# muonzoo/cutesdr

Measured on AMD Instinct MI355X. Metric: complex IQ MSamples/s through CFastFIR+demod chain; achieved HBM GB/s vs peak, higher is better.
Workload: dtype f32; 1 GPU; C3: 256 channels/GPU x 2^19 IQ samples, 16384-pt CFastFIR overlap-save (8193 taps, hop 8192), shared -5..+5 kHz filter @62.5 kS/s; channels_per_gpu=256, samples_per_channel=524288, fft_size=16384, parallelism=channels sharded x1, no data-path collective

## Files before the change

### __graft_entry__.py

```python
import os
import sys

ROOT = os.path.dirname(os.path.abspath(__file__))
if ROOT not in sys.path:
    sys.path.insert(0, ROOT)


def build():
    from cutesdr_amd import _build, _capi
    lib = _build.build()
    assert os.path.exists(lib)
    assert os.path.exists(_build.alt_lib(*_build.TWREG3))
    assert os.path.exists(_build.alt_lib(*_build.PWRES0))
    from oracle import oracle as orc
    orc.build()
    from oracle import ref
    ref.build()
    import ctypes
    L = ctypes.CDLL(lib)
    missing = [n for n in _capi.declared_symbols() if not hasattr(L, n)]
    assert not missing, missing
    import cutesdr_amd


def smoke():
    import numpy as np
    import cutesdr_amd as ca
    from oracle import oracle as orc
    n, C, fs = 16384, 4, 62500.0
    T = 3 * (n // 2)
    rng = np.random.default_rng(0)
    x = 3000.0 * (rng.standard_normal((C, T)) + 1j * rng.standard_normal((C, T)))
    b = ca.FastFirBatch(C, n, device=0)
    b.setup(-5000, 5000, 0, fs)
    y = b.process(x)
    for c in range(C):
        ff = orc.CFastFIR(n)
        ff.SetupParameters(-5000, 5000, 0, fs)
        ref = ff.ProcessData(x[c])
        err = np.abs(y[c] - ref).max()
        assert err <= 2e-5 * np.abs(x[c]).max(), err
    print("smoke ok: fastfir 16384-pt x %d channels, max err %.3g" % (C, err))


if __name__ == "__main__":
    build()
    if "--smoke" in sys.argv:
        smoke()
```

### cutesdr_amd/_build.py

```python
import glob
import os
import shutil
import subprocess
import sys

HERE = os.path.dirname(os.path.abspath(__file__))
CSRC = os.path.join(HERE, "csrc")
OBJ = os.path.join(HERE, "_obj")
LIB = os.path.join(HERE, "libcutesdr_mi.so")
ARCH = "gfx950"
FLAGS = ["-O3", "-std=c++17", "-fPIC", "--offload-arch=" + ARCH, "-Wall", "-Wno-unused-function"] + \
    os.environ.get("CSDR_EXTRA_HIPCC_FLAGS", "").split()
FILE_FLAGS = {"fastfir2_kernels.hip": ["-mllvm", "-amdgpu-sched-strategy=max-ilp"] + os.environ.get("CSDR_K1_FLAGS", "").split(), "fastfir_kernels.hip": ["-mllvm", "-amdgpu-sched-strategy=max-ilp"],
              "spectrum_kernels.hip": ["-mllvm", "-amdgpu-sched-strategy=max-ilp"]}


def _difference(text):
    import re
    m = re.fullmatch(r"\(?\s*([0-9.]+)\s*-\s*([0-9.]+)\s*\)?", text.strip())
    if not m:
        raise ValueError("unexpected threshold expression in csdr_hb_taps.h: %r" % text)
    return float(m.group(1)) - float(m.group(2))


# ... 139 lines not shown
                    r[4].kill()
                raise RuntimeError("hipcc failed on %s:\n%s" % (src, out.decode(errors="replace")))
            with open(stamp, "w") as f:
                f.write(flags)

    for src, obj, extra, stamp, flags in todo:
        reap(JOBS - 1)
        cmd = [hipcc] + FLAGS + FILE_FLAGS.get(os.path.basename(src), []) + extra + ["-c", src, "-o", obj]
        if verbose:
            print(" ".join(cmd), file=sys.stderr)
        p = subprocess.Popen(cmd, stdout=subprocess.PIPE, stderr=subprocess.STDOUT)
        running.append((src, obj, stamp, flags, p))
        procs.append(obj)
    reap(0)
    if force or procs or _newer(LIB, objs):
        cmd = [hipcc, "-shared", "-fPIC", "--offload-arch=" + ARCH, "-o", LIB] + list(link_extra) + objs
        subprocess.check_call(cmd)
    return LIB


def alt_path(name):
    return os.path.join(HERE, "libcutesdr_mi_%s.so" % name)


def alt_lib(name, extra, units=("fastfir2_kernels",), verbose=False):
    build(verbose=verbose)
    hipcc = _hipcc()
    headers = glob.glob(os.path.join(CSRC, "*.h")) + glob.glob(os.path.join(CSRC, "*.hpp")) + \
        glob.glob(os.path.join(HERE, "..", "include", "*.h"))
    out = alt_path(name)
    alt, fresh = [], False
    for unit in units:
        src = os.path.join(CSRC, unit + ".hip")
        obj = os.path.join(OBJ, "%s.%s.o" % (unit, name))
        cmd = [hipcc] + FLAGS + FILE_FLAGS.get(unit + ".hip", []) + ["-I", OBJ] + list(extra) + ["-c", src, "-o", obj]
        stamp, flags = obj + ".flags", " ".join(cmd[1:-4])
        if _newer(obj, [src] + headers) or not os.path.exists(stamp) or open(stamp).read() != flags:
            if verbose:
                print(" ".join(cmd), file=sys.stderr)
            subprocess.check_call(cmd)
            with open(stamp, "w") as f:
                f.write(flags)
            fresh = True
        alt.append(obj)
    objs = [o for o in sorted(glob.glob(os.path.join(OBJ, "*.hip.o")) + glob.glob(os.path.join(OBJ, "downconv_plan_*.o")))
            if os.path.basename(o)[:-6] not in units]
    if fresh or _newer(out, objs + alt):
        subprocess.check_call([hipcc, "-shared", "-fPIC", "--offload-arch=" + ARCH, "-o", out] + objs + alt)
    return out


TWREG3 = ("twreg3", ["-DK1_TWREG=3"])
PWRES0 = ("pwres0", ["-DK1_PWRES=0"])


if __name__ == "__main__":
    kind = next((a.split("=", 1)[1] for a in sys.argv if a.startswith("--sanitize=")), None)
    var = next((a.split("=", 1)[1] for a in sys.argv if a.startswith("--variant=")), None)
    print(build(force="--force" in sys.argv, verbose=True, sanitize=kind, variant=var,
                variant_flags=[a for a in sys.argv[1:] if a.startswith("-D")]))
```

### cutesdr_amd/csrc/capi_fastfir.hip

```cpp
#include "capi_common.hpp"
#include "capi_internal.hpp"
#include <algorithm>
#include "fastfir_kernels.h"
#include "fastfir_design_kernels.h"
#include "host_math.hpp"
#include "patch_queue.hpp"
#include <cmath>
#include <cstdlib>
#include <cstring>
#include <vector>

using namespace csdr;

static int log2_of(int n)
{
    int l = 0;
    while ((1 << l) < n) l++;
    return ((1 << l) == n) ? l : -1;
}

struct csdr_fastfir_batch {
    int device, channels, n, log2n;
    int cus;
    hipStream_t last_stream;
// ... 377 lines not shown
    else {
        b->last_kernel = FASTFIR_KERNEL_NONE;
        CSDR_HIP(fastfir_launch(b->log2n, a, s));
        b->last_kernel = FASTFIR_KERNEL_GENERIC;
    }
    b->hist_cur ^= 1;
    return CSDR_OK;
}

int csdr__fastfir_batch_copy_row(csdr_fastfir_batch *dst, int dr, csdr_fastfir_batch *src, int sr)
{
    if (!dst || !src || dst->n != src->n || dr < 0 || dr >= dst->channels || sr < 0 || sr >= src->channels)
        return fail(CSDR_EINVAL, "bad argument");
    if (!device_ok(dst->device)) return CSDR_EHIP;
    CSDR_HIP(hipDeviceSynchronize());
    const int L = dst->n / 2;
    const size_t shalf = (size_t)src->channels * L * 2, dhalf = (size_t)dst->channels * L * 2;
    CSDR_HIP(hipMemcpy(dst->d_hist + dst->hist_cur * dhalf + (size_t)dr * L * 2,
                       src->d_hist + src->hist_cur * shalf + (size_t)sr * L * 2, (size_t)L * 8, hipMemcpyDeviceToDevice));
    const int sslot = src->per_channel ? sr : 0;
    { const int rcm = fetch_mirror(src, sslot); if (rcm) return rcm; }
    const std::vector<cd> &H = src->resp[sslot];
    if (dst->channels > 1 && !dst->per_channel) return fail(CSDR_ESTATE, "destination rows share one filter");
    const int slot = dst->per_channel ? dr : 0;
    int rc = set_response(dst, slot, H);
    if (rc) return rc;
    dst->own_design = dst->own_design && src->own_design;
    dst->flo = dst->fhi = dst->off = dst->fs = std::nan("");
    return CSDR_OK;
}

int csdr__fastfir_set_variant(csdr_fastfir_batch *b, int variant)
{
    if (!b || (variant != 0 && variant != 2)) return CSDR_EINVAL;
    b->variant = variant;
    return CSDR_OK;
}

int csdr__fastfir_set_own_design(csdr_fastfir_batch *b, int own)
{
    if (!b) return CSDR_EINVAL;
    b->own_design = own != 0;
    return CSDR_OK;
}

int csdr__fastfir_last_kernel(const csdr_fastfir_batch *b, int *kernel, int *twreg)
{
    if (!b || !kernel || !twreg) return CSDR_EINVAL;
    *kernel = b->last_kernel;
    *twreg = fastfir2_twreg();
    return CSDR_OK;
}

int csdr__dbg_fastfir_stage(csdr_fastfir_batch *b, int stage, float *d_dbg)
{
    if (!b) return CSDR_EINVAL;
    b->dbg_stage = stage; b->dbg_out = d_dbg;
    return CSDR_OK;
}

}

struct csdr_fastfir {
    csdr_fastfir_batch *b;
    int n, pending;
    PinnedBuf pin_in, pin_out;
    hipStream_t s = nullptr;
    float *d_in, *d_out;
    size_t cap;
};

static int ensure_cap(csdr_fastfir *f, size_t samples)
{
    if (samples <= f->cap) return CSDR_OK;
    if (f->d_in) (void)hipFree(f->d_in);
    if (f->d_out) (void)hipFree(f->d_out);
    f->d_in = f->d_out = nullptr; f->cap = 0;
    CSDR_HIP(hipMalloc((void **)&f->d_in, samples * 8));
    CSDR_HIP(hipMalloc((void **)&f->d_out, samples * 8));
    f->cap = samples;
    return CSDR_OK;
}

extern "C" {

csdr_fastfir *csdr_fastfir_create(int device, int fft_size)
{
    csdr_fastfir_batch *b = csdr_fastfir_batch_create(device, 1, fft_size);
    if (!b) return nullptr;
    csdr_fastfir *f = new csdr_fastfir();
    f->b = b; f->n = fft_size; f->pending = 0; f->d_in = f->d_out = nullptr; f->cap = 0;
    if (hipStreamCreateWithFlags(&f->s, hipStreamNonBlocking) != hipSuccess) { csdr_fastfir_destroy(f); fail(CSDR_EHIP, "stream creation failed"); return nullptr; }
    return f;
}

void csdr_fastfir_destroy(csdr_fastfir *f)
{
    if (!f) return;
    (void)hipSetDevice(f->b->device);
    if (f->d_in) (void)hipFree(f->d_in);
    if (f->d_out) (void)hipFree(f->d_out);
    if (f->s) { (void)hipStreamSynchronize(f->s); (void)hipStreamDestroy(f->s); }
    csdr_fastfir_batch_destroy(f->b);
    delete f;
}

// ... 37 lines not shown
```

### cutesdr_amd/csrc/capi_hosttest.hip

```cpp
#include "capi_common.hpp"
#include "host_math.hpp"
#include "dc_host.hpp"
#include "pc_host.hpp"
#include "display_plan.hpp"
#include "testgen_host.hpp"
#include "scope_host.hpp"
#include "plotter_host.hpp"
#include "seq_host.hpp"
#include "spurcal_host.hpp"
#include "nb_host.hpp"
#include "fastfir_kernels.h"
#include "fft_core.hpp"
#include <cstring>

using namespace csdr;

template <int SIGN> static void host_head4_gain(const float *x4, const float *g4, float *out4)
{
    v2f x[4];
    for (int q = 0; q < 4; q++) x[q] = v2f{x4[2 * q], x4[2 * q + 1]};
    dit_head4_gain<0, 4, SIGN>(x, v2f{g4[0], g4[1]}, v2f{g4[2], g4[3]});
    for (int q = 0; q < 4; q++) { out4[2 * q] = x[q].x; out4[2 * q + 1] = x[q].y; }
}
template <int R, int SIGN> static void host_dft_middle(const float *in, float *out)
// ... 10 lines not shown
    int done = -1;
    static_for<0, R / 4>([&](auto I) {
        if (I.value != i) return;
        constexpr int Q = R / 4;
        v2f x[R];
        for (int p = 0; p < R; p++) x[p] = v2f{0.0f, 0.0f};
        for (int q = 0; q < 4; q++) x[I.value + q * Q] = v2f{in4[2 * q], in4[2 * q + 1]};
        if (middle) dit_tail_middle_r4<I.value, R, SIGN>(x); else dit_tail_r4<I.value, R, SIGN>(x);
        for (int q = 0; q < 4; q++) { out4[2 * q] = x[I.value + q * Q].x; out4[2 * q + 1] = x[I.value + q * Q].y; }
        done = 0;
    });
    return done;
}
template <int R, int SIGN> static void host_dft_r4(int middle, const float *in, float *out)
{
    v2f x[R];
    for (int n = 0; n < R; n++) x[bitrev<R>(n)] = v2f{in[2 * n], in[2 * n + 1]};
    static_for<0, R / 4>([&](auto G) { dit_head4<G.value, R, SIGN>(x); });
    if constexpr (R == 32) dit_single<8, 32, SIGN>(x);
    if (middle) {
        static_for<0, R / 4>([&](auto I) { dit_tail_middle_r4<I.value, R, SIGN>(x); });
        for (int r = 0; r < R / 2; r++) { out[2 * r] = x[R / 4 + r].x; out[2 * r + 1] = x[R / 4 + r].y; }
    } else {
        static_for<0, R / 4>([&](auto I) { dit_tail_r4<I.value, R, SIGN>(x); });
        for (int r = 0; r < R; r++) { out[2 * r] = x[r].x; out[2 * r + 1] = x[r].y; }
    }
}

extern "C" {

int csdr__host_dit_tail_r4(int r, int sign, int i, int middle, const float *in4, float *out4)
{
    if (r == 16) return sign > 0 ? host_tail_r4<16, +1>(i, middle, in4, out4) : host_tail_r4<16, -1>(i, middle, in4, out4);
    if (r == 32) return sign > 0 ? host_tail_r4<32, +1>(i, middle, in4, out4) : host_tail_r4<32, -1>(i, middle, in4, out4);
    return -1;
}
int csdr__host_dft_r4(int r, int sign, int middle, const float *in, float *out)
{
    if (r == 16 && sign > 0) host_dft_r4<16, +1>(middle, in, out);
    else if (r == 16) host_dft_r4<16, -1>(middle, in, out);
    else if (r == 32 && sign > 0) host_dft_r4<32, +1>(middle, in, out);
    else if (r == 32) host_dft_r4<32, -1>(middle, in, out);
    else return -1;
    return 0;
}
int csdr__host_tw_factors(int k, int sign, double *m, double *tau)
{
    const TwFactors f = tw_factors(k, sign);
    *m = f.m; *tau = f.tau;
    return f.rot;
}
int csdr__host_fastfir2_radix4(void) { return fastfir2_radix4(); }
int csdr__host_fastfir2_pwres(void) { return fastfir2_pwres(); }

int csdr__host_fastfir_design(int n, double flo, double fhi, double off, double fs, double *h_out)
{
    std::vector<cd> H;
    if (!fastfir_design(n, flo, fhi, off, fs, H)) return -1;
    memcpy(h_out, H.data(), sizeof(cd) * n);
    return 0;
}
int csdr__host_design_job(double flo, double fhi, double off, double fs, double *nfc, double *nfs)
{
    return fastfir_design_job(flo, fhi, off, fs, *nfc, *nfs) ? 0 : -1;
}
int csdr__host_fastfir_bin_of(int log2n, int t, int r) { return fastfir_bin_of(log2n, t, r); }
int csdr__host_fastfir_gains(int n, double flo, double fhi, double off, double fs, double *h_out, double *p_out)
{
    std::vector<cd> H;
    if (!fastfir_design(n, flo, fhi, off, fs, H)) return -1;
    memcpy(h_out, H.data(), sizeof(cd) * n);
    for (int k = 0; k < n; k++) p_out[k] = fastfir_gain(H[k], k);
    return 0;
}
int csdr__host_fastfir2_bin_of(int log2n, int t, int j, int e) { return fastfir2_bin_of(log2n, t, j, e); }
int csdr__host_fastfir2_gain_bin_of(int log2n, int t, int i, int c) { return fastfir2_gain_bin_of(log2n, t, i, c); }
int csdr__host_fastfir2_slot_bin(int log2n, int t, int j, int e) { return fastfir2_slot_bin(log2n, t, j, e); }
int csdr__host_fastfir2_gain_slot_bin(int log2n, int t, int i, int c) { return fastfir2_gain_slot_bin(log2n, t, i, c); }
void csdr__host_fastfir2_twshare_shift(int log2n, int t, int *inner, int *outer) { fastfir2_twshare_shift(log2n, t, inner, outer); }
int csdr__host_fastfir2_twshare(void) { return fastfir2_twshare(); }

void csdr__host_dit_head4_gain(int sign, const float *x4, const float *g4, float *out4)
{
    if (sign > 0) host_head4_gain<+1>(x4, g4, out4); else host_head4_gain<-1>(x4, g4, out4);
}
int csdr__host_dft_middle(int r, int sign, const float *in, float *out)
{
    if (r == 16 && sign > 0) host_dft_middle<16, +1>(in, out);
    else if (r == 16) host_dft_middle<16, -1>(in, out);
    else if (r == 32 && sign > 0) host_dft_middle<32, +1>(in, out);
    else if (r == 32) host_dft_middle<32, -1>(in, out);
    else return -1;
    return 0;
}

int csdr__host_dc_plan(double in_rate, double bw, int *codes, double *out_rate, int *warmup)
{
    DcPlan p = dc_make_plan(in_rate, bw);
    for (int i = 0; i < p.nstages; i++) codes[i] = p.kind[i];
    *out_rate = p.out_rate; *warmup = p.W;
    return p.nstages;
}
int csdr__host_dc_stage_taps(double in_rate, double bw, int s, double *h)
{
    DcPlan p = dc_make_plan(in_rate, bw);
    if (s < 0 || s >= p.nstages) return -1;
// ... 320 lines not shown
```

### cutesdr_amd/csrc/fastfir2_kernels.hip

```cpp
#define CSDR_FMA_BFLY 1
#define CSDR_PLAIN_CONST_FMA 1
#include "launch_once.hpp"
#include "fastfir_dev.hpp"
#include "fastfir_kernels.h"

namespace csdr {

#ifndef K1_LDAUX
#define K1_LDAUX 2
#endif
#ifndef K1_STAUX
#define K1_STAUX 2
#endif
#ifndef K1_HREG
#define K1_HREG 8
#endif
#ifndef K1_TWREG
#define K1_TWREG 16
#endif
#ifndef K1_HREG4K
#define K1_HREG4K 4
#endif
#ifndef K1_W1_FETCH_MAX_R0
#define K1_W1_FETCH_MAX_R0 2
#endif
#ifndef K1_HREG2K
#define K1_HREG2K 8
#endif
#ifndef K1_RADIX4
#define K1_RADIX4 1
#endif
#ifndef K1_PWRES
#define K1_PWRES 1
#endif
static_assert(K1_TWREG >= 0 && K1_TWREG <= 16, "K1_TWREG");

#define CSDR_SB() __builtin_amdgcn_sched_barrier(0)

#define CSDR_PRIO(p) __builtin_amdgcn_s_setprio(p)

#ifdef CSDR_K1_STAMPS
#define CSDR_STAMP(i)                                                                         \
    do {                                                                                      \
        CSDR_SB();                                                                            \
        unsigned long long now_;                                                              \
        asm volatile("s_memtime %0\n\ts_waitcnt lgkmcnt(0)" : "=s"(now_)::"memory");         \
        CSDR_SB();                                                                            \
        acc_[i] += now_ - last_;                                                              \
        last_ = now_;                                                                         \
    } while (0)
#define CSDR_STAMP_PARAMS , unsigned long long (&acc_)[16], unsigned long long &last_
#define CSDR_STAMP_ARGS , acc_, last_
#else
#define CSDR_STAMP(i) do { } while (0)
#define CSDR_STAMP_PARAMS
#define CSDR_STAMP_ARGS
#endif

template <int I> using int_c = std::integral_constant<int, I>;

template <int NG, class Compute, class Store> __device__ __forceinline__ void one_group_behind(Compute &&compute, Store &&store)
{
    static_for<0, NG + 1>([&](auto I) {
        constexpr int i = I.value;
        if constexpr (i < NG) compute(I);
        if constexpr (i > 0) {
            CSDR_STORE_GROUP_BEGIN();
            store(int_c<i - 1>{});
            CSDR_STORE_GROUP_END();
        } else {
            CSDR_SB();
        }
    });
}
template <int NG, class Compute, class Store> __device__ __forceinline__ void one_group_behind_st8(Compute &&compute, Store &&store)
{
    static_for<0, NG + 1>([&](auto I) {
        constexpr int i = I.value;
        if constexpr (i < NG) compute(I);
        if constexpr (i > 0) store(int_c<i - 1>{});
        CSDR_SB();
    });
}

constexpr int tws_group(int step) { return step < 2 ? 4 * step : ((step & 1) ? 8 - step / 2 : step / 2); }
constexpr int tws_set(int step) { return step < 2 ? step : 1 + step / 2; }
constexpr bool tws_opens(int step) { return step < 2 || (step & 1) == 0; }
constexpr int tws_row(int set, int slot)
{
    if (set < 2) return slot < 2 ? 8 - 4 * set + 8 * slot : 0;
    const int m = set - 1;
    return slot == 0 ? m : (slot == 1 ? m + 8 : (slot == 2 ? 8 - m : 16 - m));
}
constexpr int tws_row_of(int k1) { return k1 <= 16 ? k1 : 32 - k1; }
constexpr int tws_set_of(int k1)
{
    const int r = tws_row_of(k1) & 7;
    return r == 0 ? 0 : (r == 4 ? 1 : 1 + (r < 4 ? r : 8 - r));
}
constexpr int tws_slot_of(int k1)
{
    for (int slot = 0; slot < 4; slot++)
        if (tws_row(tws_set_of(k1), slot) == tws_row_of(k1)) return slot;
    return -1;
}
static_assert(tws_group(2) == 1 && tws_group(3) == 7 && tws_group(7) == 5 && tws_set(7) == 4 && tws_set_of(31) == 2 &&
              tws_slot_of(24) == 0 && tws_slot_of(16) == 1 && tws_slot_of(20) == 1 && tws_slot_of(25) == 2 && tws_slot_of(23) == 1,
              "twiddle sets of the 16384-point kernels");

template <int LOG2N, bool RG = false>
struct K1Cfg {
    using Base = FastFirCfg<LOG2N>;
    static_assert(!RG || LOG2N == 14, "the quarter-block shift is whole rows of the outer pass at N = 16384 only");
    static constexpr int VW = LOG2N == 12 ? 2 : (LOG2N == 11 ? 4 : 1);
    static constexpr int TV = Base::T;
    static constexpr int T = VW * TV;
    static constexpr int LDS_BYTES = (VW * Base::LDS_DATA + 1024) * 8;

    static constexpr int N = Base::N, R0 = Base::R0, G = Base::G, L = N / 2, HALF = R0 / 2;
    static_assert(R0 == 16 || R0 == 8 || R0 == 4 || R0 == 2, "the grouped outer pass is written for N = 2048 ... 16384");
    static constexpr int PSTEP = 2 * TV, PSTEP_LDS = PSTEP + 2 * (PSTEP / 32), PSTEP_B = PSTEP * 8;
    static constexpr int OUTER_ROW = 1024 + 2 * (1024 / 32);
    static constexpr bool TWS = LOG2N == 14;
    static constexpr int PWN = R0 == 16 ? R0 / 2 + 1 : R0;
    static constexpr bool W1_RESIDENT = R0 > K1_W1_FETCH_MAX_R0;
    static constexpr int HREG = RG ? 0 : (LOG2N == 12 ? K1_HREG4K : (LOG2N == 11 ? K1_HREG2K : K1_HREG));
    static constexpr int TWREG = RG ? K1_TWREG : 0;
    static constexpr bool R4 = RG && K1_RADIX4 != 0;
    static constexpr bool PW_RESIDENT = RG && K1_PWRES != 0;

    using Y = v2f[G][R0];
    using W1 = v2f[R0 > 2 ? G : 1];
    using Pw = v2f[G][PWN];
    using Hv = v4f[RG ? 1 : 16];
    using Pv = v4f[RG ? 8 : 1];
    using Twr = v2f[TWREG > 0 ? TWREG : 1];
};

struct K1Half { v2f v[16]; };

struct K1Thread {
    int t, voff;
    v2f *col;
    const v2f *twc;
    v2f *rowp;
    v2f *outer;
    const v2f_h *tw1;
    int nblocks;
    rsrc_t r_in, r_h, r_out;
#ifdef K1_ABLATE
    v4f habl;
    v2f twabl;
#endif
};

#ifdef K1_ABLATE
__device__ __forceinline__ void keep_alive(v4f v) { asm volatile("" ::"v"(v)); }
#endif

template <int LOG2N> __device__ __forceinline__ void k1_block_barrier()
{
#ifdef ABL_BAR
    wave_sync();
#else
    if constexpr (LOG2N == 11) wave_sync();
    else __syncthreads();
#endif
}

template <int LOG2N, bool RG, int K1> __device__ __forceinline__ v2f k1_pass_tw(const K1Thread &c, const typename K1Cfg<LOG2N, RG>::Twr &twr)
{
#ifdef ABL_TW
    return c.twabl;
#else
    if constexpr (K1 <= K1Cfg<LOG2N, RG>::TWREG) return twr[K1 - 1];
    else return lds_ld8(c.twc + 32 * K1);
#endif
}

template <int LOG2N, int J> __device__ __forceinline__ void k1_fetch_h(const K1Thread &c, typename K1Cfg<LOG2N>::Hv &hv)
{
#ifdef ABL_H
    hv[J] = c.habl;
#else
    if constexpr (J >= K1Cfg<LOG2N>::HREG) hv[J] = buf_load16(c.r_h, c.t * 16, J * (K1Cfg<LOG2N>::TV * 16));
#endif
}

template <int LOG2N> __device__ __forceinline__ void k1_store_out(const K1Thread &c, int voff, int soff, v4f v)
{
#ifdef ABL_GST
    if constexpr (LOG2N == 14) { keep_alive(v); return; }
#endif
    buf_store16_aux<K1_STAUX>(c.r_out, voff, soff, v);
}

template <int LOG2N> __device__ __forceinline__ void k1_load_half(rsrc_t r, int voff, int soff, v2f (&dst)[16])
{
    using Cfg = K1Cfg<LOG2N>;
#pragma unroll
    for (int n1 = 0; n1 < Cfg::HALF; n1++)
#pragma unroll
        for (int pp = 0; pp < Cfg::G / 2; pp++) {
            v4f v = buf_load16_aux<K1_LDAUX>(r, voff + pp * Cfg::PSTEP_B, soff + n1 * 8192);
            dst[(2 * pp) * Cfg::HALF + n1] = v2f{v.x, v.y};
            dst[(2 * pp + 1) * Cfg::HALF + n1] = v2f{v.z, v.w};
        }
}

template <int LOG2N> __device__ __forceinline__ v4f k1_w_pair(const K1Thread &c, int pp)
{
    return *reinterpret_cast<const v4f *>(c.tw1 + K1Cfg<LOG2N>::PSTEP * pp + 2 * c.t);
}
template <int LOG2N> __device__ __forceinline__ void k1_load_w1(const K1Thread &c, typename K1Cfg<LOG2N>::W1 &w1)
{
    if constexpr (K1Cfg<LOG2N>::R0 > 2) {
#pragma unroll
        for (int pp = 0; pp < K1Cfg<LOG2N>::G / 2; pp++) { const v4f v = k1_w_pair<LOG2N>(c, pp); w1[2 * pp] = v2f{v.x, v.y}; w1[2 * pp + 1] = v2f{v.z, v.w}; }
    }
}

template <int LOG2N, bool RG> __device__ __forceinline__ void k1_f1_rows16(const K1Thread &c, typename K1Cfg<LOG2N>::Y &y, typename K1Cfg<LOG2N>::Pw &pw)
{
    using Cfg = K1Cfg<LOG2N>;
    constexpr int R0 = Cfg::R0;
    v4f wv[16];
    one_group_behind<R0 / 4>([&](auto Ii) {
        constexpr int i = Ii.value;
        dit_tail_sel<K1Cfg<LOG2N, RG>::R4, i, R0, +1>(y[0]);
        dit_tail_sel<K1Cfg<LOG2N, RG>::R4, i, R0, +1>(y[1]);
        static_for<0, 4>([&](auto P) {
            constexpr int k0 = i + 4 * P.value;
            if constexpr (k0 > R0 / 2) {
                y[0][k0] = cmul_conj(y[0][k0], pw[0][R0 - k0]);
                y[1][k0] = cmul_conj(y[1][k0], pw[1][R0 - k0]);
            } else if constexpr (k0 != 0) {
                y[0][k0] = cmul(y[0][k0], pw[0][k0]);
                y[1][k0] = cmul(y[1][k0], pw[1][k0]);
            }
            wv[k0] = store_operand(y[0][k0], y[1][k0]);
        });
    }, [&](auto Ii) {
        static_for<0, 4>([&](auto P) {
            constexpr int k0 = Ii.value + 4 * P.value;
            *reinterpret_cast<v4f *>(c.outer + Cfg::OUTER_ROW * k0) = wv[k0];
        });
    });
}
template <int LOG2N> __device__ __forceinline__ void k1_f1_rows2(const K1Thread &c, typename K1Cfg<LOG2N>::Y &y)
{
    using Cfg = K1Cfg<LOG2N>;
    v4f wv[16], wq[8];
    static_for<0, 8>([&](auto PP) { wq[PP.value] = k1_w_pair<LOG2N>(c, PP.value); });
    one_group_behind<4>([&](auto Ii) {
        static_for<0, 2>([&](auto Q) {
            constexpr int pp = 2 * Ii.value + Q.value;
            y[2 * pp][1] = cmul(y[2 * pp][1], v2f{wq[pp].x, wq[pp].y});
            y[2 * pp + 1][1] = cmul(y[2 * pp + 1][1], v2f{wq[pp].z, wq[pp].w});
            wv[pp] = store_operand(y[2 * pp][0], y[2 * pp + 1][0]);
            wv[8 + pp] = store_operand(y[2 * pp][1], y[2 * pp + 1][1]);
// ... 2 lines not shown
        static_for<0, 2>([&](auto Q) {
            constexpr int pp = 2 * Ii.value + Q.value;
            *reinterpret_cast<v4f *>(c.outer + Cfg::PSTEP_LDS * pp) = wv[pp];
            *reinterpret_cast<v4f *>(c.outer + Cfg::OUTER_ROW + Cfg::PSTEP_LDS * pp) = wv[8 + pp];
        });
    });
}
template <int LOG2N> __device__ __forceinline__ void k1_f1_rows84(const K1Thread &c, typename K1Cfg<LOG2N>::Y &y, typename K1Cfg<LOG2N>::Pw &pw)
{
    using Cfg = K1Cfg<LOG2N>;
    constexpr int R0 = Cfg::R0, G = Cfg::G, NG = 4, RPG = R0 / NG;
    v4f wv[16];
    one_group_behind<NG>([&](auto Ii) {
        constexpr int i = Ii.value;
        if constexpr (R0 == 8)
            static_for<0, G>([&](auto E) { bfly_dit<4 * i, +1>(y[E.value][i], y[E.value][i + 4]); });
        static_for<0, RPG>([&](auto P) {
            constexpr int k0 = i + NG * P.value;
            static_for<0, G>([&](auto E) {
                if constexpr (k0 != 0) y[E.value][k0] = cmul(y[E.value][k0], pw[E.value][k0]);
            });
            static_for<0, G / 2>([&](auto PP) {
                wv[k0 * (G / 2) + PP.value] = store_operand(y[2 * PP.value][k0], y[2 * PP.value + 1][k0]);
            });
        });
    }, [&](auto Ii) {
        static_for<0, RPG>([&](auto P) {
            constexpr int k0 = Ii.value + NG * P.value;
            static_for<0, G / 2>([&](auto PP) {
                *reinterpret_cast<v4f *>(c.outer + Cfg::OUTER_ROW * k0 + Cfg::PSTEP_LDS * PP.value) = wv[k0 * (G / 2) + PP.value];
            });
        });
    });
}
template <int LOG2N, bool RG> __device__ __forceinline__ void k1_pass_f1(const K1Thread &c, int b, K1Half &oldh, K1Half &newh, typename K1Cfg<LOG2N>::Pw &pw)
{
    using Cfg = K1Cfg<LOG2N>;
    constexpr int R0 = Cfg::R0, G = Cfg::G, HALF = Cfg::HALF;
    typename Cfg::Y y;
    static_for<0, HALF>([&](auto N1) {
        static_for<0, G>([&](auto E) {
            constexpr int e = E.value, n1 = N1.value, po = bitrev<R0>(n1), pn = bitrev<R0>(HALF + n1);
            y[e][po] = oldh.v[e * HALF + n1]; y[e][pn] = newh.v[e * HALF + n1];
        });
    });
    if constexpr (R0 == 2) {
        static_for<0, G>([&](auto E) { bfly_dit<0, +1>(y[E.value][0], y[E.value][1]); });
    } else {
        static_for<0, (R0 >= 8 ? R0 / 4 : 1)>([&](auto Gg) {
            static_for<0, G>([&](auto E) { dit_head4<Gg.value, R0, +1>(y[E.value]); });
        });
    }
    CSDR_SB();
    k1_load_half<LOG2N>(c.r_in, c.voff, (b + 1 < c.nblocks ? b + 1 : c.nblocks - 1) * (Cfg::L * 8), oldh.v);
    CSDR_SB();
    CSDR_PRIO(0);
    if constexpr (R0 == 16) k1_f1_rows16<LOG2N, RG>(c, y, pw);
    else if constexpr (R0 == 2) k1_f1_rows2<LOG2N>(c, y);
    else k1_f1_rows84<LOG2N>(c, y, pw);
}

template <int LOG2N, bool RG>
__device__ __forceinline__ void k1_f2_tail_shared(const K1Thread &c, v2f (&x)[32], typename K1Cfg<LOG2N, RG>::Hv &hv,
                                                  const typename K1Cfg<LOG2N, RG>::Twr &twr CSDR_STAMP_PARAMS)
{
    v2f tw[5][4];
    auto load_set = [&](auto S) {
        static_for<0, 4>([&](auto Q) {
            constexpr int row = tws_row(S.value, Q.value);
            if constexpr (row != 0) tw[S.value][Q.value] = k1_pass_tw<LOG2N, RG, row>(c, twr);
        });
    };
    load_set(int_c<0>{});
    CSDR_SB();
    CSDR_STAMP(8);
    one_group_behind_st8<8>([&](auto St) {
        constexpr int s = St.value, i = tws_group(s);
        if constexpr (s < 7 && tws_opens(s + 1)) load_set(int_c<tws_set(s + 1)>{});
        if constexpr (!RG) { k1_fetch_h<LOG2N, 2 * s>(c, hv); k1_fetch_h<LOG2N, 2 * s + 1>(c, hv); }
        dit_tail_sel<K1Cfg<LOG2N, RG>::R4, i, 32, +1>(x);
        static_for<0, 4>([&](auto P) {
            constexpr int k1 = i + 8 * P.value;
            if constexpr (k1 != 0 && k1 <= 16) x[k1] = cmul(x[k1], tw[tws_set_of(k1)][tws_slot_of(k1)]);
            if constexpr (k1 > 16) x[k1] = cmul_conj(x[k1], tw[tws_set_of(k1)][tws_slot_of(k1)]);
        });
    }, [&](auto St) {
        static_for<0, 4>([&](auto P) {
            constexpr int k1 = tws_group(St.value) + 8 * P.value;
            lds_st8(c.col + 34 * k1, x[k1]);
        });
    });
}
template <int LOG2N, bool RG>
__device__ __forceinline__ void k1_f2_tail_plain(const K1Thread &c, v2f (&x)[32], typename K1Cfg<LOG2N, RG>::Hv &hv,
                                                 const typename K1Cfg<LOG2N, RG>::Twr &twr CSDR_STAMP_PARAMS)
{
    v2f tw[2][4];
    static_for<1, 4>([&](auto P) { tw[0][P.value] = k1_pass_tw<LOG2N, RG, 8 * P.value>(c, twr); });
    CSDR_SB();
    CSDR_STAMP(8);
    one_group_behind_st8<8>([&](auto Ii) {
        constexpr int i = Ii.value;
        if constexpr (i < 7)
            static_for<0, 4>([&](auto P) { tw[(i + 1) & 1][P.value] = k1_pass_tw<LOG2N, RG, i + 1 + 8 * P.value>(c, twr); });
        if constexpr (!RG) { k1_fetch_h<LOG2N, 2 * i>(c, hv); k1_fetch_h<LOG2N, 2 * i + 1>(c, hv); }
        dit_tail<i, 32, +1>(x);
        static_for<0, 4>([&](auto P) {
// ... 235 lines not shown
            constexpr int g = Gg.value;
            static_for<0, G>([&](auto E) {
                constexpr int e = E.value;
                if constexpr (R0 == 16) {
                    constexpr int ka = bitrev<R0>(4 * g), kb = bitrev<R0>(4 * g + 1), kc = bitrev<R0>(4 * g + 2), kd = bitrev<R0>(4 * g + 3);
                    constexpr int H0 = R0 / 2;
                    dit_head4_seltw<g, R0, -1, g == 0, (ka <= H0), (kb <= H0), (kc <= H0), (kd <= H0)>(
                        y[e], pw[e][ka <= H0 ? ka : R0 - ka], pw[e][kb <= H0 ? kb : R0 - kb],
                        pw[e][kc <= H0 ? kc : R0 - kc], pw[e][kd <= H0 ? kd : R0 - kd]);
                } else
                    dit_head4_conjtw<g, R0, -1, g == 0>(y[e], pw[e][bitrev<R0>(4 * g)], pw[e][bitrev<R0>(4 * g + 1)],
                                                        pw[e][bitrev<R0>(4 * g + 2)], pw[e][bitrev<R0>(4 * g + 3)]);
            });
            if constexpr ((g & 1) == 1) CSDR_SB();
        });
    }
    CSDR_PRIO(2);
    if constexpr (R0 == 16) k1_i3_rows16<LOG2N, RG>(c, b, y);
    else if constexpr (R0 == 2) k1_i3_rows2<LOG2N>(c, b, y);
    else k1_i3_rows84<LOG2N>(c, b, y);
}

template <int LOG2N, bool RG> __device__ __forceinline__ void fastfir_os2_body(const FastFirArgs a)
{
    CSDR_WG_TRACE_SCOPE(a.trace, WGT_FF);
    using Cfg = K1Cfg<LOG2N, RG>;
    constexpr int N = Cfg::N, T = Cfg::TV, G = Cfg::G, L = Cfg::L, HALF = Cfg::HALF, VW = Cfg::VW;
    extern __shared__ __attribute__((aligned(16))) unsigned char smem_raw[];
    const int t = VW == 1 ? (int)threadIdx.x : (int)threadIdx.x % T, vw = VW == 1 ? 0 : (int)threadIdx.x / T;
    v2f *lds = reinterpret_cast<v2f *>(smem_raw) + vw * Cfg::Base::LDS_DATA;
    v2f *tw2 = reinterpret_cast<v2f *>(smem_raw) + VW * Cfg::Base::LDS_DATA;
    if constexpr (VW > 1) {
        for (int i = threadIdx.x; i < 1024; i += VW * T) tw2[i] = a.tw2[i];
        __syncthreads();
    }

    int wg = blockIdx.x * VW + vw, ch, run;
    if ((a.channels & 7) == 0) {
        int xcd = wg & 7, slot = wg >> 3;
        ch = (slot / a.runs) * 8 + xcd;
        run = slot % a.runs;
    } else {
        ch = wg / a.runs;
        run = wg % a.runs;
    }
    const int b0 = run * a.blocks_per_run;
    int b1 = b0 + a.blocks_per_run;
    if (b1 > a.nblocks) b1 = a.nblocks;
#if defined(__HIP_DEVICE_COMPILE__) && !defined(__gfx950__)
#error "fastfir_os2_kernel<12> relies on gfx950's s_barrier ignoring terminated waves (two virtual workgroups per workgroup)"
#endif
    if (ch >= a.channels || b0 >= b1) return;

    if constexpr (VW == 1)
        for (int i = t; i < 1024; i += T) tw2[i] = a.tw2[i];

    K1Thread c;
    c.t = t; c.tw1 = a.tw1; c.nblocks = a.nblocks;
    c.r_in = make_rsrc(a.in + (long)ch * a.in_stride, (unsigned)a.nblocks * L * 8u);
    const rsrc_t r_hist = make_rsrc(a.hist + (long)ch * L, L * 8u);
    c.r_out = make_rsrc(a.out + (long)ch * a.out_stride, (unsigned)a.nblocks * L * 8u);
    c.r_h = make_rsrc(a.h + (long)ch * a.h_stride, N * 8u);
    const rsrc_t r_g = make_rsrc(a.gain + (long)ch * (a.h_stride / 2), N * 4u);
    c.voff = t * 16;

    typename Cfg::W1 w1;
    k1_load_w1<LOG2N>(c, w1);
    typename Cfg::Pw pw;
    if constexpr (Cfg::R0 > 2) {
#pragma unroll
        for (int e = 0; e < G; e++) twiddle_powers<Cfg::PWN>(opaque(w1[e]), pw[e]);
    }

    typename Cfg::Hv hv;
#pragma unroll
    for (int j = 0; j < Cfg::HREG; j++) hv[j] = buf_load16(c.r_h, t * 16, j * (T * 16));
    typename Cfg::Pv pv;
    if constexpr (RG) {
#pragma unroll
        for (int i = 0; i < 8; i++) pv[i] = buf_load16(r_g, t * 16, i * (T * 16));
    }
#ifdef K1_ABLATE
    c.habl = v4f{1.0f, 0.0f, 1.0f, 0.0f};
    asm volatile("" : "+v"(c.habl));
    c.twabl = v2f{0.8f, 0.6f};
    asm volatile("" : "+v"(c.twabl));
#endif
    v2f x[32];
    K1Half hp, hq;
    if (b0 == 0) k1_load_half<LOG2N>(r_hist, c.voff, 0, hp.v);
    else k1_load_half<LOG2N>(c.r_in, c.voff, (b0 - 1) * (L * 8), hp.v);
    k1_load_half<LOG2N>(c.r_in, c.voff, b0 * (L * 8), hq.v);

    const int sb = t >> 5, sn = t & 31;
    c.col = lds + lds_pad(1024 * sb) + sn;
    c.twc = tw2 + sn;
    typename Cfg::Twr twr;
#pragma unroll
    for (int k1 = 1; k1 <= Cfg::TWREG; k1++) twr[k1 - 1] = a.tw2[32 * k1 + sn];
    c.rowp = lds + 34 * t;
    c.outer = lds + lds_pad(2 * t);

#ifdef K1_CYC
    const unsigned long long cyc0_ = __builtin_amdgcn_s_memtime(), rt0_ = __builtin_amdgcn_s_memrealtime();
#endif
#ifdef CSDR_K1_STAMPS
    unsigned long long acc_[16] = {0, 0, 0, 0, 0, 0, 0, 0, 0, 0, 0, 0, 0, 0, 0, 0}, last_;
    asm volatile("s_memtime %0\n\ts_waitcnt lgkmcnt(0)" : "=s"(last_)::"memory");
#endif
    auto one_block = [&](const int b, K1Half &oldh, K1Half &newh) {
        CSDR_SB();
        CSDR_PRIO(1);
        k1_pass_f1<LOG2N, RG>(c, b, oldh, newh, pw);
        CSDR_STAMP(0);
        k1_block_barrier<LOG2N>();
        CSDR_STAMP(1);
        CSDR_PRIO(3);
        k1_pass_f2<LOG2N, RG>(c, x, hv, twr CSDR_STAMP_ARGS);
        CSDR_STAMP(2);
        wave_sync();
        CSDR_PRIO(2);
        k1_pass_f3<LOG2N, RG>(c, x, hv, pv);
        CSDR_STAMP(3);
        wave_sync();
        CSDR_PRIO(0);
        k1_pass_i2<LOG2N, RG>(c, x, twr);
        CSDR_STAMP(4);
        k1_block_barrier<LOG2N>();
        CSDR_STAMP(5);
        CSDR_PRIO(3);
        k1_pass_i3<LOG2N, RG>(c, b, w1, pw);
        CSDR_STAMP(6);
    };
    __builtin_amdgcn_s_waitcnt(0x0f70);
    int b = b0;
    for (; b + 1 < b1; b += 2) {
        one_block(b, hp, hq);
        one_block(b + 1, hq, hp);
    }
    const bool odd_tail = b < b1;
    if (odd_tail) one_block(b, hp, hq);

#ifdef K1_CYC
    if (a.dbg && t == 0) {
        unsigned long long *o = reinterpret_cast<unsigned long long *>(a.dbg) + (long)blockIdx.x * 2;
        o[0] = __builtin_amdgcn_s_memtime() - cyc0_;
        o[1] = __builtin_amdgcn_s_memrealtime() - rt0_;
    }
#endif
#ifdef CSDR_K1_STAMPS
    if (a.dbg && (c.t & 63) == 0) {
        unsigned long long *o = reinterpret_cast<unsigned long long *>(a.dbg) + ((long)blockIdx.x * (T / 64) + (c.t >> 6)) * 16;
        for (int i = 0; i < 16; i++) o[i] = acc_[i];
    }
#endif
    if (b1 == a.nblocks) {
        const rsrc_t r_hn = make_rsrc(a.hist_next + (long)ch * L, L * 8u);
        v4f sv[8];
#pragma unroll
        for (int n1 = 0; n1 < HALF; n1++)
#pragma unroll
            for (int pp = 0; pp < G / 2; pp++)
                sv[n1 * (G / 2) + pp] = odd_tail ? store_operand(hq.v[(2 * pp) * HALF + n1], hq.v[(2 * pp + 1) * HALF + n1])
                                                 : store_operand(hp.v[(2 * pp) * HALF + n1], hp.v[(2 * pp + 1) * HALF + n1]);
        CSDR_STORE_GROUP_BEGIN();
#pragma unroll
        for (int n1 = 0; n1 < HALF; n1++)
#pragma unroll
            for (int pp = 0; pp < G / 2; pp++) buf_store16(r_hn, c.voff + pp * Cfg::PSTEP_B, n1 * 8192, sv[n1 * (G / 2) + pp]);
        CSDR_STORE_GROUP_END();
    }
}


template <int LOG2N>
__global__ __launch_bounds__(K1Cfg<LOG2N>::T) __attribute__((amdgpu_waves_per_eu(2, 2)))
void fastfir_os2_kernel(FastFirArgs a)
{
    fastfir_os2_body<LOG2N, LOG2N == 14>(a);
}
__global__ __launch_bounds__(K1Cfg<14>::T) __attribute__((amdgpu_waves_per_eu(2, 2)))
void fastfir_os2h_kernel(FastFirArgs a)
{
    fastfir_os2_body<14, false>(a);
}

template <int LOG2N>
static hipError_t launch2_one(const FastFirArgs &a, hipStream_t stream, int *which)
{
    using Cfg = K1Cfg<LOG2N>;
    void (*kernel)(FastFirArgs) = &fastfir_os2_kernel<LOG2N>;
    if (LOG2N == 14 && !a.gain) kernel = &fastfir_os2h_kernel;
    if (which) *which = (LOG2N == 14 && kernel != &fastfir_os2h_kernel) ? FASTFIR_KERNEL_PIPELINED_GAIN : FASTFIR_KERNEL_PIPELINED_H;
    hipError_t e = kernel == &fastfir_os2h_kernel ? CSDR_MAX_LDS_ONCE(&fastfir_os2h_kernel, Cfg::LDS_BYTES)
                                                  : CSDR_MAX_LDS_ONCE(&fastfir_os2_kernel<LOG2N>, Cfg::LDS_BYTES);
    if (e != hipSuccess) return e;
#ifdef CSDR_WG_TRACE
    FastFirArgs b = a;
    b.trace = wgtrace_next();
    hipLaunchKernelGGL(kernel, dim3((a.channels * a.runs + Cfg::VW - 1) / Cfg::VW), dim3(Cfg::T), Cfg::LDS_BYTES, stream, b);
    return hipGetLastError();
#endif
    hipLaunchKernelGGL(kernel, dim3((a.channels * a.runs + Cfg::VW - 1) / Cfg::VW), dim3(Cfg::T), Cfg::LDS_BYTES, stream, a);
    return hipGetLastError();
}

hipError_t fastfir2_launch(int log2n, const FastFirArgs &a, hipStream_t stream, int *kernel)
{
    switch (log2n) {
    case 11: return launch2_one<11>(a, stream, kernel);
    case 12: return launch2_one<12>(a, stream, kernel);
    case 13: return launch2_one<13>(a, stream, kernel);
    case 14: return launch2_one<14>(a, stream, kernel);
    default: return hipErrorInvalidValue;
    }
}

int fastfir2_twreg() { return K1_TWREG; }
int fastfir2_radix4() { return K1Cfg<14, true>::R4 ? 1 : 0; }
int fastfir2_pwres() { return K1Cfg<14, true>::PW_RESIDENT ? 1 : 0; }

int fastfir2_bin_of(int log2n, int t, int j, int e)
{
    const int R0 = (1 << log2n) / 1024;
    const int i = j >> 1, h = j & 1;
    const int k2 = i + 8 * h + 16 * e;
    return (t >> 5) + R0 * ((t & 31) + 32 * k2);
}
int fastfir2_gain_bin_of(int log2n, int t, int i, int c)
{
    return fastfir2_bin_of(log2n, t, 2 * i + (c >> 1), c & 1);
}

int fastfir2_twshare() { return 2; }
void fastfir2_twshare_shift(int log2n, int t, int *inner, int *outer)
{
    *inner = (log2n == 14 && (t & 31) >= 17) ? 1 : 0;
    *outer = (log2n == 14 && (t >> 5) > 8) ? 1 : 0;
}
int fastfir2_slot_bin(int log2n, int t, int j, int e)
{
    const int R0 = (1 << log2n) / 1024;
    int inner, outer;
    fastfir2_twshare_shift(log2n, t, &inner, &outer);
    const int k2 = ((j >> 1) + 8 * (j & 1) + 16 * e - inner) & 31;
    const int sub = ((t & 31) + 32 * k2 - outer) & 1023;
    return (t >> 5) + R0 * sub;
}
int fastfir2_gain_slot_bin(int log2n, int t, int i, int c)
{
    return fastfir2_slot_bin(log2n, t, 2 * i + (c >> 1), c & 1);
}

}
```

### cutesdr_amd/csrc/fastfir_kernels.h

```cpp
#pragma once
#include <hip/hip_runtime.h>
#include "wg_trace.hpp"

namespace csdr {

typedef float v2f_h __attribute__((ext_vector_type(2)));
typedef float v4f_h __attribute__((ext_vector_type(4)));

struct FastFirArgs {
    const v2f_h *in;
    const v2f_h *hist;
    v2f_h *hist_next;
    v2f_h *out;
    const v4f_h *h;
    const v4f_h *gain;
    const v2f_h *tw1;
    const v2f_h *tw2;
    long in_stride;
    long out_stride;
    long h_stride;
    int channels;
    int nblocks;
    int blocks_per_run;
    int runs;
    int dbg_stage;
    v2f_h *dbg;
#ifdef CSDR_WG_TRACE
    WgTraceArg trace;
#endif
};

hipError_t fastfir_launch(int log2n, const FastFirArgs &a, hipStream_t stream);
int fastfir_bin_of(int log2n, int t, int r);

enum FastFirKernel { FASTFIR_KERNEL_NONE = -1, FASTFIR_KERNEL_GENERIC = 0, FASTFIR_KERNEL_PIPELINED_H = 1, FASTFIR_KERNEL_PIPELINED_GAIN = 2 };
hipError_t fastfir2_launch(int log2n, const FastFirArgs &a, hipStream_t stream, int *kernel = nullptr);
int fastfir2_twreg();
int fastfir2_radix4();
int fastfir2_pwres();
int fastfir2_bin_of(int log2n, int t, int j, int e);
int fastfir2_gain_bin_of(int log2n, int t, int i, int c);
int fastfir2_twshare();
void fastfir2_twshare_shift(int log2n, int t, int *inner, int *outer);
int fastfir2_slot_bin(int log2n, int t, int j, int e);
int fastfir2_gain_slot_bin(int log2n, int t, int i, int c);

}
```

Baseline: 233,900 MSamples/s.

## Spread next-block prefetch across FFT passes and clamp loads at run end

Splits the next-block input prefetch into four quarters, each issued between FFT passes, so HBM loads overlap compute more evenly. With RUNEND on, the kernel stores the history tail inside the block loop and sizes the input resource so loads past the run end return zero, instead of re-reading a clamped block. It also adds optional flags that move twiddle loading into a prologue and drop the tw2 LDS table. The extra SB barriers and register pressure could hurt scheduling.

```diff
diff --git a/__graft_entry__.py b/__graft_entry__.py
--- a/__graft_entry__.py
+++ b/__graft_entry__.py
@@ -12,6 +12,8 @@
     assert os.path.exists(lib)
     assert os.path.exists(_build.alt_lib(*_build.TWREG3))
     assert os.path.exists(_build.alt_lib(*_build.PWRES0))
+    assert os.path.exists(_build.alt_lib(*_build.RUNEND0))
+    assert os.path.exists(_build.alt_lib(*_build.HBMALL))
     from oracle import oracle as orc
     orc.build()
     from oracle import ref
diff --git a/cutesdr_amd/_build.py b/cutesdr_amd/_build.py
--- a/cutesdr_amd/_build.py
+++ b/cutesdr_amd/_build.py
@@ -215,6 +215,9 @@
 
 TWREG3 = ("twreg3", ["-DK1_TWREG=3"])
 PWRES0 = ("pwres0", ["-DK1_PWRES=0"])
+HBM_KNOBS = ("K1_RUNEND", "K1_PROLOGUE", "K1_TW2LDS", "K1_LDSPREAD")
+RUNEND0 = ("runend0", ["-D%s=0" % k for k in HBM_KNOBS])
+HBMALL = ("hbmall", ["-D%s=1" % k for k in HBM_KNOBS])
 
 
 if __name__ == "__main__":
diff --git a/cutesdr_amd/csrc/capi_fastfir.hip b/cutesdr_amd/csrc/capi_fastfir.hip
--- a/cutesdr_amd/csrc/capi_fastfir.hip
+++ b/cutesdr_amd/csrc/capi_fastfir.hip
@@ -453,6 +453,16 @@
     return CSDR_OK;
 }
 
+int csdr__fastfir_read_history(csdr_fastfir_batch *b, float *out, int *cur)
+{
+    if (!b || !out || !cur) return CSDR_EINVAL;
+    if (!device_ok(b->device)) return CSDR_EHIP;
+    CSDR_HIP(hipDeviceSynchronize());
+    CSDR_HIP(hipMemcpy(out, b->d_hist, 2 * (size_t)b->channels * (b->n / 2) * 8, hipMemcpyDeviceToHost));
+    *cur = b->hist_cur;
+    return CSDR_OK;
+}
+
 int csdr__dbg_fastfir_stage(csdr_fastfir_batch *b, int stage, float *d_dbg)
 {
     if (!b) return CSDR_EINVAL;
diff --git a/cutesdr_amd/csrc/capi_hosttest.hip b/cutesdr_amd/csrc/capi_hosttest.hip
--- a/cutesdr_amd/csrc/capi_hosttest.hip
+++ b/cutesdr_amd/csrc/capi_hosttest.hip
@@ -86,6 +86,8 @@
 }
 int csdr__host_fastfir2_radix4(void) { return fastfir2_radix4(); }
 int csdr__host_fastfir2_pwres(void) { return fastfir2_pwres(); }
+int csdr__host_fastfir2_hbm_knobs(void) { return fastfir2_hbm_knobs(); }
+int csdr__host_fastfir2_gain_lds_bytes(void) { return fastfir2_gain_lds_bytes(); }
 
 int csdr__host_fastfir_design(int n, double flo, double fhi, double off, double fs, double *h_out)
 {
diff --git a/cutesdr_amd/csrc/fastfir2_kernels.hip b/cutesdr_amd/csrc/fastfir2_kernels.hip
--- a/cutesdr_amd/csrc/fastfir2_kernels.hip
+++ b/cutesdr_amd/csrc/fastfir2_kernels.hip
@@ -32,6 +32,18 @@
 #endif
 #ifndef K1_PWRES
 #define K1_PWRES 1
+#endif
+#ifndef K1_RUNEND
+#define K1_RUNEND 1
+#endif
+#ifndef K1_PROLOGUE
+#define K1_PROLOGUE 0
+#endif
+#ifndef K1_TW2LDS
+#define K1_TW2LDS 0
+#endif
+#ifndef K1_LDSPREAD
+#define K1_LDSPREAD 1
 #endif
 static_assert(K1_TWREG >= 0 && K1_TWREG <= 16, "K1_TWREG");
 
@@ -115,7 +127,6 @@
     static constexpr int VW = LOG2N == 12 ? 2 : (LOG2N == 11 ? 4 : 1);
     static constexpr int TV = Base::T;
     static constexpr int T = VW * TV;
-    static constexpr int LDS_BYTES = (VW * Base::LDS_DATA + 1024) * 8;
 
     static constexpr int N = Base::N, R0 = Base::R0, G = Base::G, L = N / 2, HALF = R0 / 2;
     static_assert(R0 == 16 || R0 == 8 || R0 == 4 || R0 == 2, "the grouped outer pass is written for N = 2048 ... 16384");
@@ -128,6 +139,11 @@
     static constexpr int TWREG = RG ? K1_TWREG : 0;
     static constexpr bool R4 = RG && K1_RADIX4 != 0;
     static constexpr bool PW_RESIDENT = RG && K1_PWRES != 0;
+    static constexpr bool TW2_LDS = !(RG && TWREG == 16 && K1_TW2LDS != 0);
+    static constexpr int LDS_BYTES = (VW * Base::LDS_DATA + (TW2_LDS ? 1024 : 0)) * 8;
+    static constexpr bool RUNEND = LOG2N == 14 && K1_RUNEND != 0;
+    static constexpr bool PROLOGUE = LOG2N == 14 && K1_PROLOGUE != 0;
+    static constexpr bool LDSPREAD = RG && K1_LDSPREAD != 0;
 
     using Y = v2f[G][R0];
     using W1 = v2f[R0 > 2 ? G : 1];
@@ -148,6 +164,10 @@
     const v2f_h *tw1;
     int nblocks;
     rsrc_t r_in, r_h, r_out;
+    const void *in;
+    unsigned in_bytes;
+    int run_end;
+    rsrc_t r_hn;
 #ifdef K1_ABLATE
     v4f habl;
     v2f twabl;
@@ -195,17 +215,46 @@
     buf_store16_aux<K1_STAUX>(c.r_out, voff, soff, v);
 }
 
-template <int LOG2N> __device__ __forceinline__ void k1_load_half(rsrc_t r, int voff, int soff, v2f (&dst)[16])
-{
-    using Cfg = K1Cfg<LOG2N>;
-#pragma unroll
-    for (int n1 = 0; n1 < Cfg::HALF; n1++)
+template <int LOG2N, int N1A = 0, int N1B = K1Cfg<LOG2N>::HALF>
+__device__ __forceinline__ void k1_load_half(rsrc_t r, int voff, int soff, v2f (&dst)[16])
+{
+    using Cfg = K1Cfg<LOG2N>;
+#pragma unroll
+    for (int n1 = N1A; n1 < N1B; n1++)
 #pragma unroll
         for (int pp = 0; pp < Cfg::G / 2; pp++) {
             v4f v = buf_load16_aux<K1_LDAUX>(r, voff + pp * Cfg::PSTEP_B, soff + n1 * 8192);
             dst[(2 * pp) * Cfg::HALF + n1] = v2f{v.x, v.y};
             dst[(2 * pp + 1) * Cfg::HALF + n1] = v2f{v.z, v.w};
         }
+}
+struct K1Next { rsrc_t r; int soff; };
+template <int LOG2N> __device__ __forceinline__ K1Next k1_next_half(const K1Thread &c, int b)
+{
+    using Cfg = K1Cfg<LOG2N>;
+    if constexpr (Cfg::RUNEND) {
+        const bool more = b + 1 < c.run_end;
+        return K1Next{make_rsrc(c.in, more ? c.in_bytes : 0u), (more ? b + 1 : b) * (Cfg::L * 8)};
+    } else {
+        return K1Next{c.r_in, (b + 1 < c.nblocks ? b + 1 : c.nblocks - 1) * (Cfg::L * 8)};
+    }
+}
+template <int LOG2N> __device__ __forceinline__ void k1_store_hist(rsrc_t r_hn, int voff, const K1Half &h)
+{
+    using Cfg = K1Cfg<LOG2N>;
+    constexpr int G = Cfg::G, HALF = Cfg::HALF;
+    v4f sv[8];
+#pragma unroll
+    for (int n1 = 0; n1 < HALF; n1++)
+#pragma unroll
+        for (int pp = 0; pp < G / 2; pp++)
+            sv[n1 * (G / 2) + pp] = store_operand(h.v[(2 * pp) * HALF + n1], h.v[(2 * pp + 1) * HALF + n1]);
+    CSDR_STORE_GROUP_BEGIN();
+#pragma unroll
+    for (int n1 = 0; n1 < HALF; n1++)
+#pragma unroll
+        for (int pp = 0; pp < G / 2; pp++) buf_store16(r_hn, voff + pp * Cfg::PSTEP_B, n1 * 8192, sv[n1 * (G / 2) + pp]);
+    CSDR_STORE_GROUP_END();
 }
 
 template <int LOG2N> __device__ __forceinline__ v4f k1_w_pair(const K1Thread &c, int pp)
@@ -314,7 +363,14 @@
         });
     }
     CSDR_SB();
-    k1_load_half<LOG2N>(c.r_in, c.voff, (b + 1 < c.nblocks ? b + 1 : c.nblocks - 1) * (Cfg::L * 8), oldh.v);
+    if constexpr (Cfg::RUNEND) {
+        if (b + 1 == c.nblocks) k1_store_hist<LOG2N>(c.r_hn, c.voff, newh);
+        CSDR_SB();
+    }
+    if constexpr (!K1Cfg<LOG2N, RG>::LDSPREAD) {
+        const K1Next nx = k1_next_half<LOG2N>(c, b);
+        k1_load_half<LOG2N>(nx.r, c.voff, nx.soff, oldh.v);
+    }
     CSDR_SB();
     CSDR_PRIO(0);
     if constexpr (R0 == 16) k1_f1_rows16<LOG2N, RG>(c, y, pw);
@@ -656,7 +712,7 @@
 #endif
     if (ch >= a.channels || b0 >= b1) return;
 
-    if constexpr (VW == 1)
+    if constexpr (VW == 1 && Cfg::TW2_LDS && !Cfg::PROLOGUE)
         for (int i = t; i < 1024; i += T) tw2[i] = a.tw2[i];
 
     K1Thread c;
@@ -667,11 +723,23 @@
     c.r_h = make_rsrc(a.h + (long)ch * a.h_stride, N * 8u);
     const rsrc_t r_g = make_rsrc(a.gain + (long)ch * (a.h_stride / 2), N * 4u);
     c.voff = t * 16;
+    if constexpr (Cfg::RUNEND) {
+        c.in = a.in + (long)ch * a.in_stride; c.in_bytes = (unsigned)a.nblocks * L * 8u; c.run_end = b1;
+        c.r_hn = make_rsrc(a.hist_next + (long)ch * L, L * 8u);
+    }
 
     typename Cfg::W1 w1;
     k1_load_w1<LOG2N>(c, w1);
     typename Cfg::Pw pw;
-    if constexpr (Cfg::R0 > 2) {
+    v2f tw2_words[1024 / T];
+    if constexpr (Cfg::PROLOGUE) {
+        if constexpr (Cfg::TW2_LDS) {
+#pragma unroll
+            for (int i = 0; i < 1024 / T; i++) tw2_words[i] = a.tw2[t + i * T];
+        }
+        CSDR_SB();
+    }
+    if constexpr (Cfg::R0 > 2 && !Cfg::PROLOGUE) {
 #pragma unroll
         for (int e = 0; e < G; e++) twiddle_powers<Cfg::PWN>(opaque(w1[e]), pw[e]);
     }
@@ -702,6 +770,15 @@
     typename Cfg::Twr twr;
 #pragma unroll
     for (int k1 = 1; k1 <= Cfg::TWREG; k1++) twr[k1 - 1] = a.tw2[32 * k1 + sn];
+    if constexpr (Cfg::PROLOGUE) {
+        CSDR_SB();
+#pragma unroll
+        for (int e = 0; e < G; e++) twiddle_powers<Cfg::PWN>(opaque(w1[e]), pw[e]);
+        if constexpr (Cfg::TW2_LDS) {
+#pragma unroll
+            for (int i = 0; i < 1024 / T; i++) tw2[t + i * T] = tw2_words[i];
+        }
+    }
     c.rowp = lds + 34 * t;
     c.outer = lds + lds_pad(2 * t);
 
@@ -715,24 +792,35 @@
     auto one_block = [&](const int b, K1Half &oldh, K1Half &newh) {
         CSDR_SB();
         CSDR_PRIO(1);
+        auto spread = [&](auto Q) {
+            if constexpr (Cfg::LDSPREAD) {
+                const K1Next nx = k1_next_half<LOG2N>(c, b);
+                k1_load_half<LOG2N, Q.value * (HALF / 4), (Q.value + 1) * (HALF / 4)>(nx.r, c.voff, nx.soff, oldh.v);
+                CSDR_SB();
+            }
+        };
         k1_pass_f1<LOG2N, RG>(c, b, oldh, newh, pw);
         CSDR_STAMP(0);
         k1_block_barrier<LOG2N>();
         CSDR_STAMP(1);
         CSDR_PRIO(3);
+        spread(int_c<0>{});
         k1_pass_f2<LOG2N, RG>(c, x, hv, twr CSDR_STAMP_ARGS);
         CSDR_STAMP(2);
         wave_sync();
         CSDR_PRIO(2);
+        spread(int_c<1>{});
         k1_pass_f3<LOG2N, RG>(c, x, hv, pv);
         CSDR_STAMP(3);
         wave_sync();
         CSDR_PRIO(0);
+        spread(int_c<2>{});
         k1_pass_i2<LOG2N, RG>(c, x, twr);
         CSDR_STAMP(4);
         k1_block_barrier<LOG2N>();
         CSDR_STAMP(5);
         CSDR_PRIO(3);
+        spread(int_c<3>{});
         k1_pass_i3<LOG2N, RG>(c, b, w1, pw);
         CSDR_STAMP(6);
     };
@@ -758,7 +846,7 @@
         for (int i = 0; i < 16; i++) o[i] = acc_[i];
     }
 #endif
-    if (b1 == a.nblocks) {
+    if constexpr (!Cfg::RUNEND) if (b1 == a.nblocks) {
         const rsrc_t r_hn = make_rsrc(a.hist_next + (long)ch * L, L * 8u);
         v4f sv[8];
 #pragma unroll
@@ -796,16 +884,17 @@
     void (*kernel)(FastFirArgs) = &fastfir_os2_kernel<LOG2N>;
     if (LOG2N == 14 && !a.gain) kernel = &fastfir_os2h_kernel;
     if (which) *which = (LOG2N == 14 && kernel != &fastfir_os2h_kernel) ? FASTFIR_KERNEL_PIPELINED_GAIN : FASTFIR_KERNEL_PIPELINED_H;
+    const int lds_bytes = kernel == &fastfir_os2h_kernel ? Cfg::LDS_BYTES : K1Cfg<LOG2N, LOG2N == 14>::LDS_BYTES;
     hipError_t e = kernel == &fastfir_os2h_kernel ? CSDR_MAX_LDS_ONCE(&fastfir_os2h_kernel, Cfg::LDS_BYTES)
-                                                  : CSDR_MAX_LDS_ONCE(&fastfir_os2_kernel<LOG2N>, Cfg::LDS_BYTES);
+                                                  : CSDR_MAX_LDS_ONCE(&fastfir_os2_kernel<LOG2N>, (K1Cfg<LOG2N, LOG2N == 14>::LDS_BYTES));
     if (e != hipSuccess) return e;
 #ifdef CSDR_WG_TRACE
     FastFirArgs b = a;
     b.trace = wgtrace_next();
-    hipLaunchKernelGGL(kernel, dim3((a.channels * a.runs + Cfg::VW - 1) / Cfg::VW), dim3(Cfg::T), Cfg::LDS_BYTES, stream, b);
+    hipLaunchKernelGGL(kernel, dim3((a.channels * a.runs + Cfg::VW - 1) / Cfg::VW), dim3(Cfg::T), lds_bytes, stream, b);
     return hipGetLastError();
 #endif
-    hipLaunchKernelGGL(kernel, dim3((a.channels * a.runs + Cfg::VW - 1) / Cfg::VW), dim3(Cfg::T), Cfg::LDS_BYTES, stream, a);
+    hipLaunchKernelGGL(kernel, dim3((a.channels * a.runs + Cfg::VW - 1) / Cfg::VW), dim3(Cfg::T), lds_bytes, stream, a);
     return hipGetLastError();
 }
 
@@ -823,6 +912,12 @@
 int fastfir2_twreg() { return K1_TWREG; }
 int fastfir2_radix4() { return K1Cfg<14, true>::R4 ? 1 : 0; }
 int fastfir2_pwres() { return K1Cfg<14, true>::PW_RESIDENT ? 1 : 0; }
+int fastfir2_hbm_knobs()
+{
+    using Cfg = K1Cfg<14, true>;
+    return (Cfg::RUNEND ? 1 : 0) | (Cfg::PROLOGUE ? 2 : 0) | (Cfg::TW2_LDS ? 0 : 4) | (Cfg::LDSPREAD ? 8 : 0);
+}
+int fastfir2_gain_lds_bytes() { return K1Cfg<14, true>::LDS_BYTES; }
 
 int fastfir2_bin_of(int log2n, int t, int j, int e)
 {
diff --git a/cutesdr_amd/csrc/fastfir_kernels.h b/cutesdr_amd/csrc/fastfir_kernels.h
--- a/cutesdr_amd/csrc/fastfir_kernels.h
+++ b/cutesdr_amd/csrc/fastfir_kernels.h
@@ -38,6 +38,8 @@
 int fastfir2_twreg();
 int fastfir2_radix4();
 int fastfir2_pwres();
+int fastfir2_hbm_knobs();
+int fastfir2_gain_lds_bytes();
 int fastfir2_bin_of(int log2n, int t, int j, int e);
 int fastfir2_gain_bin_of(int log2n, int t, int i, int c);
 int fastfir2_twshare();
```

New measurement: 236,500 MSamples/s (median of 6 runs). 1.01x the previous value.
